# DeepMETv2/DeepMETv2

Measured on AMD Instinct MI355X. Metric: events/sec (4.5k PF cands, k=16), higher is better.
Workload: dtype f32

## Files before the change

deepmetv2_amd/build.py:

```python
from __future__ import annotations

import concurrent.futures as cf
import os
import shutil
import subprocess
import sys

PKG_DIR = os.path.dirname(os.path.abspath(__file__))
CSRC = os.path.join(PKG_DIR, "csrc")
OBJ_DIR = os.path.join(CSRC, "_obj")
LIB_PATH = os.path.join(PKG_DIR, "libdmet_hip.so")
SOURCES = ["knn.hip", "radius.hip", "edgeconv.hip", "edgemlp.hip", "misc.hip", "dense.hip", "encoder.hip", "norm.hip", "edgeconv_bwd.hip",
           "head.hip", "finalize.hip", "pool.hip",
           "edgemlp_f32.hip", "edgemlp_bf16.hip", "edgeconv_sum.hip", "gravnet.hip", "attention.hip", "fps.hip", "interpolate.hip",
           "pointnet.hip", "gat.hip", "segment.hip", "multi_aggr.hip", "weighted_sum.hip", "event_norm.hip", "select.hip",
           "voxel.hip", "edge_match.hip", "components.hip", "condense.hip"]
HEADERS = [os.path.join(CSRC, h) for h in ("common.h", "bn_affine.h", "knn_common.h", "knn_filter.h", "knn_key64.h", "knn_tile_schedule.h",
                                           "nls_body.h",
                                           "edgemlp_fused.h", "row_softmax.h", "score_key.h")] + \
          [os.path.join(PKG_DIR, "..", "include", "dmet.h")]
ARCH = "gfx950"
CXXFLAGS = ["-O3", "-std=c++17", "-fPIC", f"--offload-arch={ARCH}", "-ffp-contract=off", "-Wall",
            "-Wno-unused-function", "-DNDEBUG"]


def _hipcc() -> str:
    exe = shutil.which("hipcc") or "/opt/rocm/bin/hipcc"
    if not os.path.exists(exe):
        raise RuntimeError("hipcc not found: cannot build libdmet_hip.so")
    return exe


def _stale(target: str, deps) -> bool:
    if not os.path.exists(target):
        return True
    t = os.path.getmtime(target)
    return any(os.path.getmtime(d) > t for d in deps if os.path.exists(d))


def _compile(src: str, force: bool) -> str:
    obj = os.path.join(OBJ_DIR, os.path.splitext(src)[0] + ".o")
    path = os.path.join(CSRC, src)
    if force or _stale(obj, [path] + HEADERS):
        cmd = [_hipcc()] + CXXFLAGS + ["-c", path, "-o", obj]
        subprocess.check_call(cmd)
    return obj


def build_hip(force: bool = False, verbose: bool = False) -> str:
    os.makedirs(OBJ_DIR, exist_ok=True)
    with cf.ThreadPoolExecutor(max_workers=min(4, len(SOURCES))) as ex:
        objs = list(ex.map(lambda s: _compile(s, force), SOURCES))
    if force or _stale(LIB_PATH, objs):
        cmd = [_hipcc(), "-shared", "-fPIC", f"--offload-arch={ARCH}", "-o", LIB_PATH] + objs
        if verbose:
            print(" ".join(cmd))
        subprocess.check_call(cmd)
    return LIB_PATH


if __name__ == "__main__":
    print(build_hip(force="--force" in sys.argv, verbose=True))
```

deepmetv2_amd/csrc/encoder.hip:

```cpp
#include <stdlib.h>

#include "bn_affine.h"
#include "common.h"

namespace dmet {
namespace {

typedef float f32x16 __attribute__((ext_vector_type(16)));

#define ENC_PARAMS                                                                                                  \
    const float *__restrict__ Wc, const float *__restrict__ bc, const float *__restrict__ Wk,                      \
        const float *__restrict__ bk, const float *__restrict__ Wa, const float *__restrict__ ba,                  \
        const float *__restrict__ Echg, const float *__restrict__ Epdg, const float *__restrict__ Epv
#define ENC_ARGS Wc, bc, Wk, bk, Wa, ba, Echg, Epdg, Epv

__device__ __forceinline__ float elu(float z) { return z > 0.0f ? z : (__expf(z) - 1.0f); }

__device__ __forceinline__ void cat_indices(const int64_t *__restrict__ xcat, const float *__restrict__ row, int64_t i,
                                            int &ichg, int &ipdg, int &ipv)
{
    long long c = xcat ? xcat[i * 3 + 0] : (long long)row[8];
    const long long chg = xcat ? xcat[i * 3 + 1] : (long long)row[9];
    const long long pv = xcat ? xcat[i * 3 + 2] : (long long)row[10];
    c = c < 0 ? -c : c;
    const long long table[7] = {1, 2, 11, 13, 22, 130, 211};
#pragma unroll
    for (int t = 0; t < 7; ++t) c = (c == table[t]) ? (long long)t : c;
    ipdg = (int)min(max(c, 0ll), 6ll);
    ichg = (int)min(max(chg + 1, 0ll), 2ll);
    ipv = (int)min(max(pv, 0ll), 7ll);
}

__device__ __forceinline__ void encode_node(ENC_PARAMS, const float (&xc)[8], int ichg, int ipdg, int ipv,
                                            float (&cat24)[24], float (&z1)[16], float (&z2)[16], float (&joint)[32],
                                            float (&z3)[32])
{
#pragma unroll
    for (int e = 0; e < 8; ++e) {
        cat24[e] = Echg[ichg * 8 + e];
        cat24[8 + e] = Epdg[ipdg * 8 + e];
        cat24[16 + e] = Epv[ipv * 8 + e];
    }
#pragma unroll
    for (int o = 0; o < 16; ++o) {
        float a = bc[o];
#pragma unroll
        for (int f = 0; f < 8; ++f) a = __builtin_fmaf(Wc[o * 8 + f], xc[f], a);
        z1[o] = a;
        float b = bk[o];
#pragma unroll
        for (int f = 0; f < 24; ++f) b = __builtin_fmaf(Wk[o * 24 + f], cat24[f], b);
        z2[o] = b;
    }
#pragma unroll
    for (int o = 0; o < 16; ++o) { joint[o] = elu(z2[o]); joint[16 + o] = elu(z1[o]); }
#pragma unroll
    for (int o = 0; o < 32; ++o) {
        float a = ba[o];
#pragma unroll
        for (int f = 0; f < 32; ++f) a = __builtin_fmaf(Wa[o * 32 + f], joint[f], a);
        z3[o] = a;
    }
}

__global__ __launch_bounds__(256, 2) void encode_fwd_kernel(const float *__restrict__ x, int64_t x_stride,
                                                          const int64_t *__restrict__ xcat, int64_t N,
                                                          ENC_PARAMS, float *__restrict__ h)
{
    const int64_t i = (int64_t)blockIdx.x * blockDim.x + threadIdx.x;
    if (i >= N) return;
    const float *row = x + i * x_stride;
    float xc[8];
#pragma unroll
    for (int f = 0; f < 8; ++f) xc[f] = row[f];
    int ichg, ipdg, ipv;
    cat_indices(xcat, row, i, ichg, ipdg, ipv);
    float cat24[24], z1[16], z2[16], joint[32], z3[32];
    encode_node(ENC_ARGS, xc, ichg, ipdg, ipv, cat24, z1, z2, joint, z3);
    float4 *o = reinterpret_cast<float4 *>(h + i * 32);
#pragma unroll
    for (int c = 0; c < 8; ++c)
        o[c] = make_float4(elu(z3[4 * c]), elu(z3[4 * c + 1]), elu(z3[4 * c + 2]), elu(z3[4 * c + 3]));
}

__global__ __launch_bounds__(256) void encode_fwd_mfma_kernel(const float *__restrict__ x, int64_t x_stride,
                                                               const int64_t *__restrict__ xcat, int64_t N, ENC_PARAMS,
                                                               float *__restrict__ h)
{
    const int lane = threadIdx.x & 63, r = lane & 31, hh = lane >> 5;
    const int64_t wave = (int64_t)blockIdx.x * (blockDim.x >> 6) + __builtin_amdgcn_readfirstlane((int)(threadIdx.x >> 6));
    const int64_t nwaves = (int64_t)gridDim.x * (blockDim.x >> 6);
    const int64_t ntiles = (N + 31) / 32;
    float w12[16], w3[16], b12[16], b3[16];
#pragma unroll
    for (int s = 0; s < 16; ++s) {
        const int f = (s & 3) + 8 * (s >> 2) + 4 * hh;
        const float *src = r < 16 ? Wk + r * 24 + min(f, 23) : Wc + (r - 16) * 8 + max(f - 24, 0);
        const bool keep = r < 16 ? f < 24 : f >= 24;
        const float a = *src;
        w12[s] = keep ? a : 0.0f;
        w3[s] = Wa[r * 32 + f];
        const float *bsrc = f < 16 ? bk + f : bc + (f - 16);
        b12[s] = *bsrc;
        b3[s] = ba[f];
    }
    struct Raw { float c[4]; long long k0, k1, k2; };
    auto load_raw = [&](const int64_t tile, Raw &q) __attribute__((always_inline)) {
        const int64_t node = tile * 32 + r;
        const int64_t i = node < N ? node : N - 1;
        const float *row = x + i * x_stride;
#pragma unroll
        for (int u = 0; u < 4; ++u) q.c[u] = row[4 * hh + u];
        if (xcat) { q.k0 = xcat[i * 3 + 0]; q.k1 = xcat[i * 3 + 1]; q.k2 = xcat[i * 3 + 2]; }
        else { q.k0 = (long long)row[8]; q.k1 = (long long)row[9]; q.k2 = (long long)row[10]; }
    };
    auto load_tables = [&](const Raw &q, float (&in)[16]) __attribute__((always_inline)) {
        long long c = q.k0 < 0 ? -q.k0 : q.k0;
        const long long table[7] = {1, 2, 11, 13, 22, 130, 211};
#pragma unroll
        for (int t = 0; t < 7; ++t) c = (c == table[t]) ? (long long)t : c;
        const int ipdg = (int)min(max(c, 0ll), 6ll), ichg = (int)min(max(q.k1 + 1, 0ll), 2ll), ipv = (int)min(max(q.k2, 0ll), 7ll);
        const float4 e0 = *reinterpret_cast<const float4 *>(Echg + ichg * 8 + 4 * hh);
        const float4 e1 = *reinterpret_cast<const float4 *>(Epdg + ipdg * 8 + 4 * hh);
        const float4 e2 = *reinterpret_cast<const float4 *>(Epv + ipv * 8 + 4 * hh);
        in[0] = e0.x; in[1] = e0.y; in[2] = e0.z; in[3] = e0.w; in[4] = e1.x; in[5] = e1.y; in[6] = e1.z; in[7] = e1.w;
        in[8] = e2.x; in[9] = e2.y; in[10] = e2.z; in[11] = e2.w;
#pragma unroll
        for (int u = 0; u < 4; ++u) in[12 + u] = q.c[u];
    };
    Raw raw;
    float in[16], nxt[16];
    if (wave < ntiles) { load_raw(wave, raw); load_tables(raw, in); }
    if (wave + nwaves < ntiles) load_raw(wave + nwaves, raw);
    for (int64_t tile = wave; tile < ntiles; tile += nwaves) {
        const int64_t node = tile * 32 + r;
        if (tile + nwaves < ntiles) load_tables(raw, nxt);
        if (tile + 2 * nwaves < ntiles) load_raw(tile + 2 * nwaves, raw);
        f32x16 acc;
#pragma unroll
        for (int e = 0; e < 16; ++e) acc[e] = b12[e];
#pragma unroll
        for (int s = 0; s < 16; ++s) acc = __builtin_amdgcn_mfma_f32_32x32x2f32(w12[s], in[s], acc, 0, 0, 0);
        float joint[16];
#pragma unroll
        for (int e = 0; e < 16; ++e) joint[e] = elu(acc[e]);
#pragma unroll
        for (int e = 0; e < 16; ++e) acc[e] = b3[e];
#pragma unroll
        for (int s = 0; s < 16; ++s) acc = __builtin_amdgcn_mfma_f32_32x32x2f32(w3[s], joint[s], acc, 0, 0, 0);
        if (node < N) {
            float4 *o = reinterpret_cast<float4 *>(h + node * 32 + 4 * hh);
#pragma unroll
            for (int g = 0; g < 4; ++g)
                o[2 * g] = make_float4(elu(acc[4 * g]), elu(acc[4 * g + 1]), elu(acc[4 * g + 2]), elu(acc[4 * g + 3]));
        }
#pragma unroll
        for (int u = 0; u < 16; ++u) in[u] = nxt[u];
    }
}

constexpr int kEncTiles = 3;
constexpr int kEncBwdWaves = 4;
constexpr int kEncPartial = kEncTiles * 1024 + 64;

__device__ __forceinline__ void enc_wave_sync()
{
    __builtin_amdgcn_fence(__ATOMIC_RELEASE, "wavefront");
    __builtin_amdgcn_wave_barrier();
    __builtin_amdgcn_fence(__ATOMIC_ACQUIRE, "wavefront");
}

__device__ __forceinline__ void tile_mma(f32x16 &acc, const float *__restrict__ A, const float *__restrict__ Bm, int lane)
{
    const int c = lane & 31, hh = lane >> 5;
#pragma unroll 8
    for (int s = 0; s < 32; ++s) {
        const int node = 2 * s + hh;
        acc = __builtin_amdgcn_mfma_f32_32x32x2f32(A[node * 33 + c], Bm[node * 33 + c], acc, 0, 0, 0);
    }
}

__device__ __forceinline__ void tile_mma_onehot(f32x16 &acc, const int *__restrict__ packed, const float *__restrict__ Bm,
                                                int lane)
{
    const int c = lane & 31, hh = lane >> 5;
    int sh, mask, tgt;
    if (c < 3) { sh = 0; mask = 3; tgt = c; }
    else if (c < 10) { sh = 2; mask = 7; tgt = c - 3; }
    else if (c < 18) { sh = 5; mask = 7; tgt = c - 10; }
    else { sh = 0; mask = 0; tgt = 1; }
#pragma unroll 8
    for (int s = 0; s < 32; ++s) {
        const int node = 2 * s + hh;
        const float a = (((packed[node] >> sh) & mask) == tgt) ? 1.0f : 0.0f;
        acc = __builtin_amdgcn_mfma_f32_32x32x2f32(a, Bm[node * 33 + c], acc, 0, 0, 0);
    }
}

__device__ __forceinline__ float column_half_sum(const float *__restrict__ A, int lane)
{
    const int c = lane & 31, hh = lane >> 5;
    float s = 0.0f;
#pragma unroll 8
    for (int n = 0; n < 32; ++n) s += A[(hh * 32 + n) * 33 + c];
    return s;
}

__global__ __launch_bounds__(64 * kEncBwdWaves, 2) void encode_bwd_kernel(const float *__restrict__ x, int64_t x_stride,
                                                                          const int64_t *__restrict__ xcat, int64_t N,
                                                                          ENC_PARAMS, const float *__restrict__ gh,
                                                                          const float *__restrict__ hout,
                                                                          int64_t nodes_per_wave,
                                                                          float *__restrict__ partial)
{
    __shared__ float bufA[kEncBwdWaves][64 * 33];
    __shared__ float bufB[kEncBwdWaves][64 * 33];
    __shared__ int bufI[kEncBwdWaves][64];
    const int lane = threadIdx.x & 63, wv = __builtin_amdgcn_readfirstlane(threadIdx.x >> 6);
    float *A = bufA[wv], *Bm = bufB[wv];
    int *packed = bufI[wv];
    const int64_t wave = (int64_t)blockIdx.x * kEncBwdWaves + wv;
    const int64_t lo = wave * nodes_per_wave, hi = min(N, lo + nodes_per_wave);
    f32x16 acc[kEncTiles];
#pragma unroll
    for (int t = 0; t < kEncTiles; ++t)
#pragma unroll
        for (int e = 0; e < 16; ++e) acc[t][e] = 0.0f;
    float bias3 = 0.0f, bias21 = 0.0f;

    for (int64_t base = lo; base < hi; base += 64) {
        int zero = 0;
        asm volatile("" : "+s"(zero));
        const float *__restrict__ wc = Wc + zero, *__restrict__ wk = Wk + zero, *__restrict__ wa = Wa + zero,
                                  *__restrict__ pbc = bc + zero, *__restrict__ pbk = bk + zero;
        const int64_t i = base + lane;
        const bool live = i < hi;
        const int64_t ii = live ? i : (hi - 1);
        const float *row = x + ii * x_stride;
        float xc[8];
#pragma unroll
        for (int f = 0; f < 8; ++f) xc[f] = row[f];
        int ichg, ipdg, ipv;
        cat_indices(xcat, row, ii, ichg, ipdg, ipv);
// ... 128 lines not shown
{
    const int c = lane & 31, hh = lane >> 5;
    float s = 0.0f;
#pragma unroll 8
    for (int n = 0; n < 16; ++n) s += A[(hh * 16 + n) * 33 + c];
    return s;
}

struct EncBnBwd {
    const float *gamma, *mean, *invstd, *mean_g, *mean_gx;
};

template <bool BNB = false>
__global__ __launch_bounds__(64 * kEncBwdWaves, 2) void encode_bwd_mfma_kernel(const float *__restrict__ x, int64_t x_stride,
                                                                               const int64_t *__restrict__ xcat, int64_t N,
                                                                               ENC_PARAMS, const float *__restrict__ gh,
                                                                               const float *__restrict__ hout,
                                                                               int64_t ,
                                                                               float *__restrict__ partial,
                                                                               EncBnBwd bnb = EncBnBwd{})
{
    __shared__ float bufA[kEncBwdWaves][64 * 33];
    __shared__ float bufB[kEncBwdWaves][64 * 33];
    __shared__ int bufI[kEncBwdWaves][64];
    const int lane = threadIdx.x & 63, wv = __builtin_amdgcn_readfirstlane(threadIdx.x >> 6);
    const int r = lane & 31, hh = lane >> 5;
    float *A = bufA[wv], *Bm = bufB[wv];
    int *packed = bufI[wv];
    const int64_t wave = (int64_t)blockIdx.x * kEncBwdWaves + wv, nwaves = (int64_t)gridDim.x * kEncBwdWaves;
    const int64_t ntiles = (N + 31) / 32, hi = N;
    float w12[16], w3t[16], w12t[16], b12[16];
#pragma unroll
    for (int s = 0; s < 16; ++s) {
        const int f = (s & 3) + 8 * (s >> 2) + 4 * hh;
        {
            const float *src = r < 16 ? Wk + r * 24 + min(f, 23) : Wc + (r - 16) * 8 + max(f - 24, 0);
            const bool keep = r < 16 ? f < 24 : f >= 24;
            const float a = *src;
            w12[s] = keep ? a : 0.0f;
        }
        w3t[s] = Wa[f * 32 + r];
        {
            const float *src = f < 16 ? Wk + f * 24 + min(r, 23) : Wc + (f - 16) * 8 + max(r - 24, 0);
            const bool keep = f < 16 ? r < 24 : r >= 24;
            const float a = *src;
            w12t[s] = keep ? a : 0.0f;
        }
        const float *bsrc = f < 16 ? bk + f : bc + (f - 16);
        b12[s] = *bsrc;
    }
    f32x16 acc[kEncTiles];
#pragma unroll
    for (int t = 0; t < kEncTiles; ++t)
#pragma unroll
        for (int e = 0; e < 16; ++e) acc[t][e] = 0.0f;
    float bias3 = 0.0f, bias21 = 0.0f;

    struct Raw { float c[4]; long long k0, k1, k2; };
    auto load_raw = [&](const int64_t tile, Raw &q) __attribute__((always_inline)) {
        const int64_t nd = tile * 32 + r;
        const int64_t i = nd < N ? nd : N - 1;
        const float *row = x + i * x_stride;
#pragma unroll
        for (int u = 0; u < 4; ++u) q.c[u] = row[4 * hh + u];
        if (xcat) { q.k0 = xcat[i * 3 + 0]; q.k1 = xcat[i * 3 + 1]; q.k2 = xcat[i * 3 + 2]; }
        else { q.k0 = (long long)row[8]; q.k1 = (long long)row[9]; q.k2 = (long long)row[10]; }
    };
    auto load_tables = [&](const Raw &q, float (&in)[16], int &pk) __attribute__((always_inline)) {
        long long c = q.k0 < 0 ? -q.k0 : q.k0;
        const long long table[7] = {1, 2, 11, 13, 22, 130, 211};
#pragma unroll
        for (int t = 0; t < 7; ++t) c = (c == table[t]) ? (long long)t : c;
        const int ipdg = (int)min(max(c, 0ll), 6ll), ichg = (int)min(max(q.k1 + 1, 0ll), 2ll), ipv = (int)min(max(q.k2, 0ll), 7ll);
        pk = ichg | (ipdg << 2) | (ipv << 5);
        const float4 e0 = *reinterpret_cast<const float4 *>(Echg + ichg * 8 + 4 * hh);
        const float4 e1 = *reinterpret_cast<const float4 *>(Epdg + ipdg * 8 + 4 * hh);
        const float4 e2 = *reinterpret_cast<const float4 *>(Epv + ipv * 8 + 4 * hh);
        in[0] = e0.x; in[1] = e0.y; in[2] = e0.z; in[3] = e0.w; in[4] = e1.x; in[5] = e1.y; in[6] = e1.z; in[7] = e1.w;
        in[8] = e2.x; in[9] = e2.y; in[10] = e2.z; in[11] = e2.w;
#pragma unroll
        for (int u = 0; u < 4; ++u) in[12 + u] = q.c[u];
    };
    Raw raw;
    float in[16], nxt[16];
    int pk = 0, pk_nxt = 0;
    if (wave < ntiles) { load_raw(wave, raw); load_tables(raw, in, pk); }
    if (wave + nwaves < ntiles) load_raw(wave + nwaves, raw);
    for (int64_t tile = wave; tile < ntiles; tile += nwaves) {
        const int64_t node = tile * 32 + r;
        const bool live = node < hi;
        const int64_t ii = live ? node : (hi - 1);
        if (tile + nwaves < ntiles) load_tables(raw, nxt, pk_nxt);
        if (tile + 2 * nwaves < ntiles) load_raw(tile + 2 * nwaves, raw);
        if (hh == 0) packed[r] = pk;
        float gz[16];
        {
            const float4 *gp = reinterpret_cast<const float4 *>(gh + ii * 32 + 4 * hh);
            const float4 *hp = reinterpret_cast<const float4 *>(hout + ii * 32 + 4 * hh);
#pragma unroll
            for (int g = 0; g < 4; ++g) {
                float4 gv = gp[2 * g];
                const float4 hv = hp[2 * g];
                if constexpr (BNB) {
                    const int c0 = 8 * g + 4 * hh;
                    const float4 ga = *reinterpret_cast<const float4 *>(bnb.gamma + c0), mu = *reinterpret_cast<const float4 *>(bnb.mean + c0);
                    const float4 is = *reinterpret_cast<const float4 *>(bnb.invstd + c0), mg = *reinterpret_cast<const float4 *>(bnb.mean_g + c0);
                    const float4 mx = *reinterpret_cast<const float4 *>(bnb.mean_gx + c0);
                    gv = bn_bwd4(gv, hv, ga, mu, is, mg, mx);
                }
                const float gg[4] = {gv.x, gv.y, gv.z, gv.w}, hh4[4] = {hv.x, hv.y, hv.z, hv.w};
#pragma unroll
                for (int u = 0; u < 4; ++u) {
                    const float d = hh4[u] > 0.0f ? 1.0f : (hh4[u] + 1.0f);
                    gz[4 * g + u] = live ? gg[u] * d : 0.0f;
                }
            }
        }
        f32x16 c1;
#pragma unroll
        for (int e = 0; e < 16; ++e) c1[e] = b12[e];
#pragma unroll
        for (int s = 0; s < 16; ++s) c1 = __builtin_amdgcn_mfma_f32_32x32x2f32(w12[s], in[s], c1, 0, 0, 0);
        float joint[16];
#pragma unroll
        for (int e = 0; e < 16; ++e) joint[e] = elu(c1[e]);
#pragma unroll
        for (int e = 0; e < 16; ++e) {
            const int ch = (e & 3) + 8 * (e >> 2) + 4 * hh;
            A[r * 33 + ch] = gz[e];
            Bm[r * 33 + ch] = joint[e];
        }
        enc_lds_sync();
        tile_mma32(acc[0], A, Bm, lane);
        bias3 += column_half_sum32(A, lane);
        f32x16 c2;
#pragma unroll
        for (int e = 0; e < 16; ++e) c2[e] = 0.0f;
#pragma unroll
        for (int s = 0; s < 16; ++s) c2 = __builtin_amdgcn_mfma_f32_32x32x2f32(w3t[s], gz[s], c2, 0, 0, 0);
        float gj[16];
#pragma unroll
        for (int e = 0; e < 16; ++e) gj[e] = c2[e] * (joint[e] > 0.0f ? 1.0f : (joint[e] + 1.0f));
        enc_lds_sync();
#pragma unroll
        for (int e = 0; e < 16; ++e) {
            const int ch = (e & 3) + 8 * (e >> 2) + 4 * hh;
            A[r * 33 + ch] = gj[e];
            Bm[r * 33 + ch] = in[e];
        }
        enc_lds_sync();
        tile_mma32(acc[1], A, Bm, lane);
        bias21 += column_half_sum32(A, lane);
        f32x16 c3;
#pragma unroll
        for (int e = 0; e < 16; ++e) c3[e] = 0.0f;
#pragma unroll
        for (int s = 0; s < 16; ++s) c3 = __builtin_amdgcn_mfma_f32_32x32x2f32(w12t[s], gj[s], c3, 0, 0, 0);
        enc_lds_sync();
#pragma unroll
        for (int e = 0; e < 16; ++e) {
            const int ch = (e & 3) + 8 * (e >> 2) + 4 * hh;
            Bm[r * 33 + ch] = ch < 24 ? c3[e] : 0.0f;
        }
        enc_lds_sync();
        tile_mma_onehot32(acc[2], packed, Bm, lane);
        enc_lds_sync();
#pragma unroll
        for (int u = 0; u < 16; ++u) in[u] = nxt[u];
        pk = pk_nxt;
    }
    const int c = lane & 31;
    __syncthreads();
#pragma unroll
    for (int e = 0; e < 16; ++e) {
        const int rr = (e & 3) + 8 * (e >> 2) + 4 * hh;
        A[rr * 32 + c] = acc[0][e];
        A[1024 + rr * 32 + c] = acc[2][e];
        Bm[rr * 32 + c] = acc[1][e];
    }
    const float b3 = bias3 + __shfl_xor(bias3, 32), b21 = bias21 + __shfl_xor(bias21, 32);
    if (hh == 0) { Bm[1024 + c] = b3; Bm[1024 + 32 + c] = b21; }
    __syncthreads();
    float *out = partial + (int64_t)blockIdx.x * kEncPartial;
    for (int i = threadIdx.x; i < kEncPartial; i += 64 * kEncBwdWaves) {
        const float *src = i < 1024 ? &bufA[0][i] : i < 2048 ? &bufB[0][i - 1024] : i < 3072 ? &bufA[0][i - 1024]
                                                                                              : &bufB[0][i - 2048];
        float t = src[0];
#pragma unroll
        for (int w = 1; w < kEncBwdWaves; ++w) t += src[w * 64 * 33];
        out[i] = t;
    }
}

struct EncGrads {
    float *Wc, *bc, *Wk, *bk, *Wa, *ba, *Echg, *Epdg, *Epv;
};

__global__ __launch_bounds__(1024) void encode_bwd_finalize_kernel(const float *__restrict__ partial, int64_t nwaves,
                                                                    EncGrads g)
{
    __shared__ float red[32][33];
    const int e = threadIdx.x & 31, grp = threadIdx.x >> 5;
    const int idx = blockIdx.x * 32 + e;
    float s = 0.0f;
#pragma unroll 8
    for (int64_t w = grp; w < nwaves; w += 32) s += partial[w * kEncPartial + idx];
    red[grp][e] = s;
    __syncthreads();
    if (grp != 0) return;
    s = 0.0f;
#pragma unroll
    for (int q = 0; q < 32; ++q) s += red[q][e];
    const int t = idx / 1024, r = (idx % 1024) / 32, c = idx % 32;
    if (t == 0) g.Wa[r * 32 + c] = s;
    else if (t == 1) {
        if (r < 16 && c < 24) g.Wk[r * 24 + c] = s;
        else if (r >= 16 && c >= 24) g.Wc[(r - 16) * 8 + (c - 24)] = s;
    } else if (t == 2) {
        if (r < 3 && c < 8) g.Echg[r * 8 + c] = s;
        else if (r >= 3 && r < 10 && c >= 8 && c < 16) g.Epdg[(r - 3) * 8 + (c - 8)] = s;
        else if (r >= 10 && r < 18 && c >= 16 && c < 24) g.Epv[(r - 10) * 8 + (c - 16)] = s;
    } else if (r == 0) g.ba[c] = s;
    else if (c < 16) g.bk[c] = s;
    else g.bc[c - 16] = s;
}

inline int64_t enc_nodes_per_wave(int64_t N, int64_t *nwaves)
{
    const int64_t target_waves = 2048;
    int64_t npw = (N + target_waves - 1) / target_waves;
#ifdef DMET_ENC_NPW_UP
    npw = (npw + 63) / 64 * 64;
#else
    npw = npw / 64 * 64;
#endif
    if (npw < 64) npw = 64;
    int64_t nw = (N + npw - 1) / npw;
    nw = (nw + kEncBwdWaves - 1) / kEncBwdWaves * kEncBwdWaves;
    *nwaves = nw;
    return npw;
}

thread_local EncBnBwd g_enc_bnb{nullptr, nullptr, nullptr, nullptr, nullptr};
thread_local bool g_enc_bnb_done = false;

}
}

using namespace dmet;

extern "C" int dmet_encode_fwd_f32(const float *x, int64_t x_stride, const int64_t *xcat, int64_t N, const float *Wc, const float *bc,
                                   const float *Wk, const float *bk, const float *Wa, const float *ba,
                                   const float *Echg, const float *Epdg, const float *Epv, float *h,
                                   dmet_stream_t stream)
{
    DMET_REQUIRE(N >= 0 && x_stride >= 8, "dmet_encode_fwd_f32: bad sizes");
    if (N == 0) return 0;
    DMET_REQUIRE(x && Wc && bc && Wk && bk && Wa && ba && Echg && Epdg && Epv && h, "dmet_encode_fwd_f32: null pointer");
    DMET_REQUIRE(xcat || x_stride >= 11, "dmet_encode_fwd_f32: x_cat == NULL needs rows of at least 11 columns (x_stride=%lld)", (long long)x_stride);
    DMET_REQUIRE(aligned16(h), "dmet_encode_fwd_f32: h must be 16-B aligned");
    const int64_t blocks = (N + 255) / 256;
    DMET_REQUIRE(blocks < (1ll << 31), "dmet_encode_fwd_f32: too many nodes");
    const int form = env_is("DMET_ENCODER_FWD", "valu") ? 0 : 1;
    if (form == 1 && aligned16(Echg) && aligned16(Epdg) && aligned16(Epv)) {
        const int64_t tiles = (N + 31) / 32;
        int64_t grid = (tiles + 3) / 4;
        int gmax = 512;
        if (const char *e = getenv("DMET_ENC_GRID")) { gmax = atoi(e); if (gmax < 1) gmax = 512; }
        if (grid > gmax) grid = gmax;
        hipLaunchKernelGGL(encode_fwd_mfma_kernel, dim3((unsigned)grid), dim3(256), 0, as_stream(stream), x, x_stride, xcat, N,
                           ENC_ARGS, h);
        DMET_LAUNCH_CHECK("encode_fwd_mfma_kernel");
        return 0;
    }
    hipLaunchKernelGGL(encode_fwd_kernel, dim3((unsigned)blocks), dim3(256), 0, as_stream(stream), x, x_stride, xcat, N, ENC_ARGS, h);
    DMET_LAUNCH_CHECK("encode_fwd_kernel");
    return 0;
}

extern "C" size_t dmet_encode_bwd_workspace_bytes(int64_t N)
{
    if (N <= 0) return 0;
    int64_t nw;
    (void)enc_nodes_per_wave(N, &nw);
    return sizeof(float) * (size_t)nw * kEncPartial + 512;
}

extern "C" int dmet_encode_bwd_f32(const float *x, int64_t x_stride, const int64_t *xcat, int64_t N, const float *Wc, const float *bc,
                                   const float *Wk, const float *bk, const float *Wa, const float *ba,
                                   const float *Echg, const float *Epdg, const float *Epv, const float *h,
                                   const float *g_h, float *gWc, float *gbc, float *gWk, float *gbk, float *gWa,
                                   float *gba, float *gEchg, float *gEpdg, float *gEpv, void *ws, size_t ws_bytes,
                                   dmet_stream_t stream)
{
    DMET_REQUIRE(N > 0 && x_stride >= 8, "dmet_encode_bwd_f32: bad sizes");
    DMET_REQUIRE((xcat || x_stride >= 11) && x && Wc && bc && Wk && bk && Wa && ba && Echg && Epdg && Epv && h && g_h && gWc && gbc && gWk && gbk &&
                     gWa && gba && gEchg && gEpdg && gEpv && ws,
                 "dmet_encode_bwd_f32: null pointer");
    DMET_REQUIRE(ws_bytes >= dmet_encode_bwd_workspace_bytes(N), "dmet_encode_bwd_f32: workspace too small");
    DMET_REQUIRE(aligned16(h) && aligned16(g_h), "dmet_encode_bwd_f32: h / g_h must be 16-B aligned");
    int64_t nw;
    const int64_t npw = enc_nodes_per_wave(N, &nw);
    float *partial = reinterpret_cast<float *>((reinterpret_cast<uintptr_t>(ws) + 255u) & ~(uintptr_t)255u);
    hipStream_t st = as_stream(stream);
    const int form = env_is("DMET_ENCODER_BWD", "valu") ? 0 : 1;
    int64_t nparts = nw / kEncBwdWaves;
    if (form == 1 && aligned16(Echg) && aligned16(Epdg) && aligned16(Epv) && aligned16(g_h) && aligned16(h)) {
        const int64_t tiles = (N + 31) / 32;
        int64_t grid = (tiles + kEncBwdWaves - 1) / kEncBwdWaves;
        if (grid > 512) grid = 512;
        if (grid > nparts) grid = nparts;
        nparts = grid;
        if (g_enc_bnb.gamma)
            hipLaunchKernelGGL(encode_bwd_mfma_kernel<true>, dim3((unsigned)grid), dim3(64 * kEncBwdWaves), 0, st, x, x_stride, xcat,
                               N, ENC_ARGS, g_h, h, npw, partial, g_enc_bnb);
        else
            hipLaunchKernelGGL(encode_bwd_mfma_kernel<false>, dim3((unsigned)grid), dim3(64 * kEncBwdWaves), 0, st, x, x_stride,
                               xcat, N, ENC_ARGS, g_h, h, npw, partial, EncBnBwd{});
        g_enc_bnb_done = g_enc_bnb.gamma != nullptr;
    } else {
        hipLaunchKernelGGL(encode_bwd_kernel, dim3((unsigned)(nw / kEncBwdWaves)), dim3(64 * kEncBwdWaves), 0, st, x, x_stride,
                           xcat, N, ENC_ARGS, g_h, h, npw, partial);
    }
    DMET_LAUNCH_CHECK("encode_bwd_kernel");
    EncGrads gr{gWc, gbc, gWk, gbk, gWa, gba, gEchg, gEpdg, gEpv};
    static_assert(kEncPartial % 32 == 0, "finalize blocks own 32 elements");
    static_assert(kEncPartial == kEncPartialFloats, "csrc/finalize.hip sums the same partial layout");
    if (defer_push(DeferDesc{kDeferEncoder, partial, nparts, {gWc, gbc, gWk, gbk, gWa, gba, gEchg, gEpdg, gEpv}})) return 0;
    hipLaunchKernelGGL(encode_bwd_finalize_kernel, dim3(kEncPartial / 32), dim3(1024), 0, st, partial, nparts, gr);
    DMET_LAUNCH_CHECK("encode_bwd_finalize_kernel");
    return 0;
}

extern "C" int dmet_encode_bn_bwd_f32(const float *x, int64_t x_stride, const int64_t *xcat, int64_t N, const float *Wc,
                                      const float *bc, const float *Wk, const float *bk, const float *Wa, const float *ba,
                                      const float *Echg, const float *Epdg, const float *Epv, const float *h,
                                      const float *g_y, const float *bn_gamma, const float *bn_mean, const float *bn_invstd,
                                      const float *bn_mean_g, const float *bn_mean_gx, float *gWc, float *gbc, float *gWk,
                                      float *gbk, float *gWa, float *gba, float *gEchg, float *gEpdg, float *gEpv,
                                      int *fused, void *ws, size_t ws_bytes, dmet_stream_t stream)
{
    DMET_REQUIRE(fused, "dmet_encode_bn_bwd_f32: fused is null");
    *fused = 0;
    DMET_REQUIRE(bn_gamma && bn_mean && bn_invstd && bn_mean_g && bn_mean_gx, "dmet_encode_bn_bwd_f32: null pointer");
    const bool ok = !env_is("DMET_ENCODER_BWD", "valu") && N > 0 && aligned16(Echg) && aligned16(Epdg) && aligned16(Epv) && aligned16(g_y) &&
                    aligned16(h) && aligned16(bn_gamma) && aligned16(bn_mean) && aligned16(bn_invstd) && aligned16(bn_mean_g) &&
                    aligned16(bn_mean_gx);
    if (!ok) return 0;
    g_enc_bnb = EncBnBwd{bn_gamma, bn_mean, bn_invstd, bn_mean_g, bn_mean_gx};
    g_enc_bnb_done = false;
    const int rc = dmet_encode_bwd_f32(x, x_stride, xcat, N, Wc, bc, Wk, bk, Wa, ba, Echg, Epdg, Epv, h, g_y, gWc, gbc, gWk, gbk, gWa,
                                       gba, gEchg, gEpdg, gEpv, ws, ws_bytes, stream);
    const bool done = g_enc_bnb_done;
    g_enc_bnb = EncBnBwd{nullptr, nullptr, nullptr, nullptr, nullptr};
    g_enc_bnb_done = false;
    if (rc == 0 && !done) {
        set_error("dmet_encode_bn_bwd_f32: the matrix-core backward it was checked for did not run");
        return -22;
    }
    *fused = rc == 0 ? 1 : 0;
    return rc;
}
```

Measured before the change: 53370.

## Add two-stream interleaved MFMA encoder kernels and move bwd prefetch later

Adds forward and backward encoder kernels in which each wavefront processes two node tiles at once, interleaving their MFMA chains with the ELU/VALU work of the other stream to hide dependency latency. A shared node-tile schedule header is introduced. The new kernels are opt-in via DMET_NODE_STREAMS=2. The existing backward kernel is also changed to prefetch the next tile's tables after the LDS stage instead of holding a separate nxt buffer, which saves registers but makes the loads later in the loop.

```diff
diff --git a/deepmetv2_amd/build.py b/deepmetv2_amd/build.py
--- a/deepmetv2_amd/build.py
+++ b/deepmetv2_amd/build.py
@@ -16,7 +16,7 @@
            "pointnet.hip", "gat.hip", "segment.hip", "multi_aggr.hip", "weighted_sum.hip", "event_norm.hip", "select.hip",
            "voxel.hip", "edge_match.hip", "components.hip", "condense.hip"]
 HEADERS = [os.path.join(CSRC, h) for h in ("common.h", "bn_affine.h", "knn_common.h", "knn_filter.h", "knn_key64.h", "knn_tile_schedule.h",
-                                           "nls_body.h",
+                                           "nls_body.h", "node_tile_schedule.h",
                                            "edgemlp_fused.h", "row_softmax.h", "score_key.h")] + \
           [os.path.join(PKG_DIR, "..", "include", "dmet.h")]
 ARCH = "gfx950"
diff --git a/deepmetv2_amd/csrc/encoder.hip b/deepmetv2_amd/csrc/encoder.hip
--- a/deepmetv2_amd/csrc/encoder.hip
+++ b/deepmetv2_amd/csrc/encoder.hip
@@ -2,6 +2,7 @@
 
 #include "bn_affine.h"
 #include "common.h"
+#include "node_tile_schedule.h"
 
 namespace dmet {
 namespace {
@@ -159,6 +160,151 @@
     }
 }
 
+struct EncRaw { float c[4]; long long k0, k1, k2; };
+
+__device__ __forceinline__ void enc_load_raw(const float *__restrict__ x, int64_t x_stride, const int64_t *__restrict__ xcat,
+                                             int64_t N, int64_t tile, int r, int hh, EncRaw &q)
+{
+    const int64_t i = node_row(tile, r, N);
+    const float *row = x + i * x_stride;
+#pragma unroll
+    for (int u = 0; u < 4; ++u) q.c[u] = row[4 * hh + u];
+    if (xcat) { q.k0 = xcat[i * 3 + 0]; q.k1 = xcat[i * 3 + 1]; q.k2 = xcat[i * 3 + 2]; }
+    else { q.k0 = (long long)row[8]; q.k1 = (long long)row[9]; q.k2 = (long long)row[10]; }
+}
+
+__device__ __forceinline__ void enc_load_tables(const float *__restrict__ Echg, const float *__restrict__ Epdg,
+                                                const float *__restrict__ Epv, int hh, const EncRaw &q, float (&in)[16], int &pk)
+{
+    long long c = q.k0 < 0 ? -q.k0 : q.k0;
+    const long long table[7] = {1, 2, 11, 13, 22, 130, 211};
+#pragma unroll
+    for (int t = 0; t < 7; ++t) c = (c == table[t]) ? (long long)t : c;
+    const int ipdg = (int)min(max(c, 0ll), 6ll), ichg = (int)min(max(q.k1 + 1, 0ll), 2ll), ipv = (int)min(max(q.k2, 0ll), 7ll);
+    pk = ichg | (ipdg << 2) | (ipv << 5);
+    const float4 e0 = *reinterpret_cast<const float4 *>(Echg + ichg * 8 + 4 * hh);
+    const float4 e1 = *reinterpret_cast<const float4 *>(Epdg + ipdg * 8 + 4 * hh);
+    const float4 e2 = *reinterpret_cast<const float4 *>(Epv + ipv * 8 + 4 * hh);
+    in[0] = e0.x; in[1] = e0.y; in[2] = e0.z; in[3] = e0.w; in[4] = e1.x; in[5] = e1.y; in[6] = e1.z; in[7] = e1.w;
+    in[8] = e2.x; in[9] = e2.y; in[10] = e2.z; in[11] = e2.w;
+#pragma unroll
+    for (int u = 0; u < 4; ++u) in[12 + u] = q.c[u];
+}
+
+__device__ __forceinline__ void enc_pin(float &v)
+{
+    asm volatile("" : "+v"(v));
+    __builtin_amdgcn_sched_barrier(0);
+}
+
+__device__ __forceinline__ float enc_elu_here(float z)
+{
+    asm volatile("" : "+v"(z));
+    float a = elu(z);
+    enc_pin(a);
+    return a;
+}
+
+__device__ __forceinline__ void enc_pin_acc(f32x16 &c)
+{
+    asm volatile("" : "+a"(c));
+}
+
+__device__ __forceinline__ f32x16 enc_splat(const float (&b)[16])
+{
+    f32x16 a;
+#pragma unroll
+    for (int e = 0; e < 16; ++e) a[e] = b[e];
+    return a;
+}
+
+__global__ __launch_bounds__(256) void encode_fwd_mfma2_kernel(const float *__restrict__ x, int64_t x_stride,
+                                                                const int64_t *__restrict__ xcat, int64_t N, ENC_PARAMS,
+                                                                float *__restrict__ h)
+{
+    constexpr int S = kNodeStreams;
+    static_assert(S == 2, "the stages below are written out for two streams");
+    const int lane = threadIdx.x & 63, r = lane & 31, hh = lane >> 5;
+    const int64_t wavefront = (int64_t)blockIdx.x * (blockDim.x >> 6) + __builtin_amdgcn_readfirstlane((int)(threadIdx.x >> 6));
+    const int64_t nw = (int64_t)gridDim.x * (blockDim.x >> 6) * S;
+    const int64_t ntiles = node_tile_count(N);
+    float w12[16], w3[16], b12[16], b3[16];
+#pragma unroll
+    for (int s = 0; s < 16; ++s) {
+        const int f = (s & 3) + 8 * (s >> 2) + 4 * hh;
+        const float *src = r < 16 ? Wk + r * 24 + min(f, 23) : Wc + (r - 16) * 8 + max(f - 24, 0);
+        const bool keep = r < 16 ? f < 24 : f >= 24;
+        const float a = *src;
+        w12[s] = keep ? a : 0.0f;
+        w3[s] = Wa[r * 32 + f];
+        const float *bsrc = f < 16 ? bk + f : bc + (f - 16);
+        b12[s] = *bsrc;
+        b3[s] = ba[f];
+    }
+    int64_t w[S];
+    EncRaw raw[S];
+    float in[S][16], nxt[S][16];
+    int pk_unused;
+#pragma unroll
+    for (int q = 0; q < S; ++q) {
+        w[q] = node_stream_wave(wavefront, q, S);
+#pragma unroll
+        for (int u = 0; u < 16; ++u) { in[q][u] = 0.0f; nxt[q][u] = 0.0f; }
+        if (node_stream_has(w[q], 0, nw, ntiles)) enc_load_raw(x, x_stride, xcat, N, node_stream_tile(w[q], 0, nw), r, hh, raw[q]);
+    }
+#pragma unroll
+    for (int q = 0; q < S; ++q) {
+        if (node_stream_has(w[q], 0, nw, ntiles)) enc_load_tables(Echg, Epdg, Epv, hh, raw[q], in[q], pk_unused);
+        if (node_stream_has(w[q], 1, nw, ntiles)) enc_load_raw(x, x_stride, xcat, N, node_stream_tile(w[q], 1, nw), r, hh, raw[q]);
+    }
+    const int64_t rounds = node_rounds(w[0], nw, ntiles);
+    for (int64_t j = 0; j < rounds; ++j) {
+#pragma unroll
+        for (int q = 0; q < S; ++q) {
+            if (node_stream_has(w[q], j + 1, nw, ntiles)) enc_load_tables(Echg, Epdg, Epv, hh, raw[q], nxt[q], pk_unused);
+            if (node_stream_has(w[q], j + kNodePrefetch, nw, ntiles))
+                enc_load_raw(x, x_stride, xcat, N, node_stream_tile(w[q], j + kNodePrefetch, nw), r, hh, raw[q]);
+        }
+        f32x16 c1[S], c2[S];
+        float joint[S][16];
+        c1[0] = enc_splat(b12);
+#pragma unroll
+        for (int s = 0; s < 16; ++s) c1[0] = __builtin_amdgcn_mfma_f32_32x32x2f32(w12[s], in[0][s], c1[0], 0, 0, 0);
+        c1[1] = enc_splat(b12);
+#pragma unroll
+        for (int s = 0; s < 16; ++s) {
+            c1[1] = __builtin_amdgcn_mfma_f32_32x32x2f32(w12[s], in[1][s], c1[1], 0, 0, 0);
+            joint[0][s] = elu(c1[0][s]);
+        }
+        c2[0] = enc_splat(b3);
+#pragma unroll
+        for (int s = 0; s < 16; ++s) {
+            c2[0] = __builtin_amdgcn_mfma_f32_32x32x2f32(w3[s], joint[0][s], c2[0], 0, 0, 0);
+            joint[1][s] = elu(c1[1][s]);
+        }
+        c2[1] = enc_splat(b3);
+        float out0[16];
+#pragma unroll
+        for (int s = 0; s < 16; ++s) {
+            c2[1] = __builtin_amdgcn_mfma_f32_32x32x2f32(w3[s], joint[1][s], c2[1], 0, 0, 0);
+            out0[s] = elu(c2[0][s]);
+        }
+#pragma unroll
+        for (int q = 0; q < S; ++q) {
+            const int64_t tile = node_stream_tile(w[q], j, nw);
+            if (node_row_live(tile, r, N)) {
+                float4 *o = reinterpret_cast<float4 *>(h + (tile * kNodeTileRows + r) * 32 + 4 * hh);
+#pragma unroll
+                for (int g = 0; g < 4; ++g)
+                    o[2 * g] = q == 0 ? make_float4(out0[4 * g], out0[4 * g + 1], out0[4 * g + 2], out0[4 * g + 3])
+                                      : make_float4(elu(c2[1][4 * g]), elu(c2[1][4 * g + 1]), elu(c2[1][4 * g + 2]), elu(c2[1][4 * g + 3]));
+            }
+#pragma unroll
+            for (int u = 0; u < 16; ++u) in[q][u] = nxt[q][u];
+        }
+    }
+}
+
 constexpr int kEncTiles = 3;
 constexpr int kEncBwdWaves = 4;
 constexpr int kEncPartial = kEncTiles * 1024 + 64;
@@ -453,16 +599,14 @@
         for (int u = 0; u < 4; ++u) in[12 + u] = q.c[u];
     };
     Raw raw;
-    float in[16], nxt[16];
-    int pk = 0, pk_nxt = 0;
+    float in[16];
+    int pk = 0;
     if (wave < ntiles) { load_raw(wave, raw); load_tables(raw, in, pk); }
     if (wave + nwaves < ntiles) load_raw(wave + nwaves, raw);
     for (int64_t tile = wave; tile < ntiles; tile += nwaves) {
         const int64_t node = tile * 32 + r;
         const bool live = node < hi;
         const int64_t ii = live ? node : (hi - 1);
-        if (tile + nwaves < ntiles) load_tables(raw, nxt, pk_nxt);
-        if (tile + 2 * nwaves < ntiles) load_raw(tile + 2 * nwaves, raw);
         if (hh == 0) packed[r] = pk;
         float gz[16];
         {
@@ -520,6 +664,8 @@
             Bm[r * 33 + ch] = in[e];
         }
         enc_lds_sync();
+        if (tile + nwaves < ntiles) load_tables(raw, in, pk);
+        if (tile + 2 * nwaves < ntiles) load_raw(tile + 2 * nwaves, raw);
         tile_mma32(acc[1], A, Bm, lane);
         bias21 += column_half_sum32(A, lane);
         f32x16 c3;
@@ -536,9 +682,6 @@
         enc_lds_sync();
         tile_mma_onehot32(acc[2], packed, Bm, lane);
         enc_lds_sync();
-#pragma unroll
-        for (int u = 0; u < 16; ++u) in[u] = nxt[u];
-        pk = pk_nxt;
     }
     const int c = lane & 31;
     __syncthreads();
@@ -559,6 +702,252 @@
         float t = src[0];
 #pragma unroll
         for (int w = 1; w < kEncBwdWaves; ++w) t += src[w * 64 * 33];
+        out[i] = t;
+    }
+}
+
+template <int T>
+__device__ __forceinline__ void tile_mma32_streams(f32x16 (&acc)[kNodeStreams][kEncTiles], float (&bias)[kNodeStreams],
+                                                   float *const (&A)[kNodeStreams], float *const (&Bm)[kNodeStreams], int lane)
+{
+    const int c = lane & 31, hh = lane >> 5;
+    float cs[kNodeStreams];
+#pragma unroll
+    for (int q = 0; q < kNodeStreams; ++q) cs[q] = 0.0f;
+#pragma unroll
+    for (int s = 0; s < 16; ++s)
+#pragma unroll
+        for (int q = 0; q < kNodeStreams; ++q) {
+            const int node = 2 * s + hh;
+            acc[q][T] = __builtin_amdgcn_mfma_f32_32x32x2f32(A[q][node * 33 + c], Bm[q][node * 33 + c], acc[q][T], 0, 0, 0);
+            cs[q] += A[q][(hh * 16 + s) * 33 + c];
+        }
+#pragma unroll
+    for (int q = 0; q < kNodeStreams; ++q) bias[q] += cs[q];
+}
+
+__device__ __forceinline__ void tile_mma_onehot32_streams(f32x16 (&acc)[kNodeStreams][kEncTiles], int *const (&packed)[kNodeStreams],
+                                                          float *const (&Bm)[kNodeStreams], int lane)
+{
+    const int c = lane & 31, hh = lane >> 5;
+    int sh, mask, tgt;
+    if (c < 3) { sh = 0; mask = 3; tgt = c; }
+    else if (c < 10) { sh = 2; mask = 7; tgt = c - 3; }
+    else if (c < 18) { sh = 5; mask = 7; tgt = c - 10; }
+    else { sh = 0; mask = 0; tgt = 1; }
+#pragma unroll
+    for (int s = 0; s < 16; ++s)
+#pragma unroll
+        for (int q = 0; q < kNodeStreams; ++q) {
+            const int node = 2 * s + hh;
+            const float a = (((packed[q][node] >> sh) & mask) == tgt) ? 1.0f : 0.0f;
+            acc[q][2] = __builtin_amdgcn_mfma_f32_32x32x2f32(a, Bm[q][node * 33 + c], acc[q][2], 0, 0, 0);
+        }
+}
+
+template <bool BNB = false>
+__global__ __launch_bounds__(64 * kEncBwdWaves / kNodeStreams, 1) void encode_bwd_mfma2_kernel(
+    const float *__restrict__ x, int64_t x_stride, const int64_t *__restrict__ xcat, int64_t N, ENC_PARAMS,
+    const float *__restrict__ gh, const float *__restrict__ hout, float *__restrict__ partial, EncBnBwd bnb = EncBnBwd{})
+{
+    constexpr int S = kNodeStreams;
+    static_assert(S == 2 && kEncBwdWaves == kNodeBwdGroupStreams, "two wavefronts of two streams stand for the four of a partial");
+    __shared__ float bufA[kEncBwdWaves][64 * 33];
+    __shared__ float bufB[kEncBwdWaves][64 * 33];
+    __shared__ int bufI[kEncBwdWaves][64];
+    const int lane = threadIdx.x & 63, wv = __builtin_amdgcn_readfirstlane(threadIdx.x >> 6);
+    const int r = lane & 31, hh = lane >> 5;
+    const int64_t wavefront = (int64_t)blockIdx.x * (kEncBwdWaves / S) + wv;
+    const int64_t nw = (int64_t)gridDim.x * kEncBwdWaves;
+    const int64_t ntiles = node_tile_count(N);
+    float *A[S], *Bm[S];
+    int *packed[S];
+    int64_t w[S];
+#pragma unroll
+    for (int q = 0; q < S; ++q) {
+        A[q] = bufA[S * wv + q]; Bm[q] = bufB[S * wv + q]; packed[q] = bufI[S * wv + q];
+        w[q] = node_stream_wave(wavefront, q, S);
+    }
+    float w12[16], w3t[16], w12t[16], b12[16];
+#pragma unroll
+    for (int s = 0; s < 16; ++s) {
+        const int f = (s & 3) + 8 * (s >> 2) + 4 * hh;
+        {
+            const float *src = r < 16 ? Wk + r * 24 + min(f, 23) : Wc + (r - 16) * 8 + max(f - 24, 0);
+            const bool keep = r < 16 ? f < 24 : f >= 24;
+            const float a = *src;
+            w12[s] = keep ? a : 0.0f;
+        }
+        w3t[s] = Wa[f * 32 + r];
+        {
+            const float *src = f < 16 ? Wk + f * 24 + min(r, 23) : Wc + (f - 16) * 8 + max(r - 24, 0);
+            const bool keep = f < 16 ? r < 24 : r >= 24;
+            const float a = *src;
+            w12t[s] = keep ? a : 0.0f;
+        }
+        const float *bsrc = f < 16 ? bk + f : bc + (f - 16);
+        b12[s] = *bsrc;
+    }
+    f32x16 acc[S][kEncTiles];
+    float bias3[S], bias21[S];
+    EncRaw raw[S];
+    float in[S][16];
+    int pk[S];
+#pragma unroll
+    for (int q = 0; q < S; ++q) {
+#pragma unroll
+        for (int t = 0; t < kEncTiles; ++t)
+#pragma unroll
+            for (int e = 0; e < 16; ++e) acc[q][t][e] = 0.0f;
+        bias3[q] = 0.0f; bias21[q] = 0.0f; pk[q] = 0;
+#pragma unroll
+        for (int u = 0; u < 16; ++u) in[q][u] = 0.0f;
+        if (node_stream_has(w[q], 0, nw, ntiles)) enc_load_raw(x, x_stride, xcat, N, node_stream_tile(w[q], 0, nw), r, hh, raw[q]);
+    }
+#pragma unroll
+    for (int q = 0; q < S; ++q) {
+        if (node_stream_has(w[q], 0, nw, ntiles)) enc_load_tables(Echg, Epdg, Epv, hh, raw[q], in[q], pk[q]);
+        if (node_stream_has(w[q], 1, nw, ntiles)) enc_load_raw(x, x_stride, xcat, N, node_stream_tile(w[q], 1, nw), r, hh, raw[q]);
+    }
+    const int64_t rounds = node_rounds(w[0], nw, ntiles);
+    for (int64_t j = 0; j < rounds; ++j) {
+        float gz[S][16];
+        int zero = 0;
+        asm volatile("" : "+s"(zero));
+        const EncBnBwd bn{bnb.gamma + zero, bnb.mean + zero, bnb.invstd + zero, bnb.mean_g + zero, bnb.mean_gx + zero};
+#pragma unroll
+        for (int q = 0; q < S; ++q) {
+            if (hh == 0) packed[q][r] = pk[q];
+        }
+        bool live[S];
+        const float4 *gp[S], *hp[S];
+#pragma unroll
+        for (int q = 0; q < S; ++q) {
+            const int64_t tile = node_stream_tile(w[q], j, nw);
+            live[q] = node_row_live(tile, r, N);
+            const int64_t ii = node_row(tile, r, N);
+            gp[q] = reinterpret_cast<const float4 *>(gh + ii * 32 + 4 * hh);
+            hp[q] = reinterpret_cast<const float4 *>(hout + ii * 32 + 4 * hh);
+        }
+#pragma unroll
+        for (int g = 0; g < 4; ++g) {
+            float4 ga, mu, is, mg, mx;
+            if constexpr (BNB) {
+                const int c0 = 8 * g + 4 * hh;
+                ga = *reinterpret_cast<const float4 *>(bn.gamma + c0); mu = *reinterpret_cast<const float4 *>(bn.mean + c0);
+                is = *reinterpret_cast<const float4 *>(bn.invstd + c0); mg = *reinterpret_cast<const float4 *>(bn.mean_g + c0);
+                mx = *reinterpret_cast<const float4 *>(bn.mean_gx + c0);
+            }
+#pragma unroll
+            for (int q = 0; q < S; ++q) {
+                float4 gv = gp[q][2 * g];
+                const float4 hv = hp[q][2 * g];
+                if constexpr (BNB) gv = bn_bwd4(gv, hv, ga, mu, is, mg, mx);
+                const float gg[4] = {gv.x, gv.y, gv.z, gv.w}, hh4[4] = {hv.x, hv.y, hv.z, hv.w};
+#pragma unroll
+                for (int u = 0; u < 4; ++u) {
+                    const float d = hh4[u] > 0.0f ? 1.0f : (hh4[u] + 1.0f);
+                    gz[q][4 * g + u] = live[q] ? gg[u] * d : 0.0f;
+                }
+            }
+        }
+        f32x16 c1[S], c2[S], c3[S];
+        float joint[S][16], gj[S][16];
+        c1[0] = enc_splat(b12);
+#pragma unroll
+        for (int s = 0; s < 16; ++s) c1[0] = __builtin_amdgcn_mfma_f32_32x32x2f32(w12[s], in[0][s], c1[0], 0, 0, 0);
+        c1[1] = enc_splat(b12);
+#pragma unroll
+        for (int s = 0; s < 16; ++s) {
+            c1[1] = __builtin_amdgcn_mfma_f32_32x32x2f32(w12[s], in[1][s], c1[1], 0, 0, 0);
+            enc_pin_acc(c1[1]);
+            joint[0][s] = enc_elu_here(c1[0][s]);
+        }
+#pragma unroll
+        for (int e = 0; e < 16; ++e) c2[0][e] = 0.0f;
+#pragma unroll
+        for (int s = 0; s < 16; ++s) {
+            c2[0] = __builtin_amdgcn_mfma_f32_32x32x2f32(w3t[s], gz[0][s], c2[0], 0, 0, 0);
+            enc_pin_acc(c2[0]);
+            joint[1][s] = enc_elu_here(c1[1][s]);
+        }
+#pragma unroll
+        for (int e = 0; e < 16; ++e) c2[1][e] = 0.0f;
+#pragma unroll
+        for (int s = 0; s < 16; ++s) {
+            c2[1] = __builtin_amdgcn_mfma_f32_32x32x2f32(w3t[s], gz[1][s], c2[1], 0, 0, 0);
+            const int ch = (s & 3) + 8 * (s >> 2) + 4 * hh;
+            A[0][r * 33 + ch] = gz[0][s];
+            Bm[0][r * 33 + ch] = joint[0][s];
+            __builtin_amdgcn_sched_barrier(0);
+        }
+#pragma unroll
+        for (int e = 0; e < 16; ++e) {
+            const int ch = (e & 3) + 8 * (e >> 2) + 4 * hh;
+            A[1][r * 33 + ch] = gz[1][e];
+            Bm[1][r * 33 + ch] = joint[1][e];
+        }
+        enc_lds_sync();
+        tile_mma32_streams<0>(acc, bias3, A, Bm, lane);
+#pragma unroll
+        for (int q = 0; q < S; ++q)
+#pragma unroll
+            for (int e = 0; e < 16; ++e) gj[q][e] = c2[q][e] * (joint[q][e] > 0.0f ? 1.0f : (joint[q][e] + 1.0f));
+        enc_lds_sync();
+#pragma unroll
+        for (int q = 0; q < S; ++q) {
+#pragma unroll
+            for (int e = 0; e < 16; ++e) c3[q][e] = 0.0f;
+#pragma unroll
+            for (int s = 0; s < 16; ++s) {
+                c3[q] = __builtin_amdgcn_mfma_f32_32x32x2f32(w12t[s], gj[q][s], c3[q], 0, 0, 0);
+                const int ch = (s & 3) + 8 * (s >> 2) + 4 * hh;
+                A[q][r * 33 + ch] = gj[q][s];
+                Bm[q][r * 33 + ch] = in[q][s];
+            }
+        }
+        enc_lds_sync();
+#pragma unroll
+        for (int q = 0; q < S; ++q) {
+            if (node_stream_has(w[q], j + 1, nw, ntiles)) enc_load_tables(Echg, Epdg, Epv, hh, raw[q], in[q], pk[q]);
+            if (node_stream_has(w[q], j + kNodePrefetch, nw, ntiles))
+                enc_load_raw(x, x_stride, xcat, N, node_stream_tile(w[q], j + kNodePrefetch, nw), r, hh, raw[q]);
+        }
+        tile_mma32_streams<1>(acc, bias21, A, Bm, lane);
+        enc_lds_sync();
+#pragma unroll
+        for (int q = 0; q < S; ++q)
+#pragma unroll
+            for (int e = 0; e < 16; ++e) {
+                const int ch = (e & 3) + 8 * (e >> 2) + 4 * hh;
+                Bm[q][r * 33 + ch] = ch < 24 ? c3[q][e] : 0.0f;
+            }
+        enc_lds_sync();
+        tile_mma_onehot32_streams(acc, packed, Bm, lane);
+        enc_lds_sync();
+    }
+    const int c = lane & 31;
+    __syncthreads();
+#pragma unroll
+    for (int q = 0; q < S; ++q) {
+#pragma unroll
+        for (int e = 0; e < 16; ++e) {
+            const int rr = (e & 3) + 8 * (e >> 2) + 4 * hh;
+            A[q][rr * 32 + c] = acc[q][0][e];
+            A[q][1024 + rr * 32 + c] = acc[q][2][e];
+            Bm[q][rr * 32 + c] = acc[q][1][e];
+        }
+        const float b3 = bias3[q] + __shfl_xor(bias3[q], 32), b21 = bias21[q] + __shfl_xor(bias21[q], 32);
+        if (hh == 0) { Bm[q][1024 + c] = b3; Bm[q][1024 + 32 + c] = b21; }
+    }
+    __syncthreads();
+    float *out = partial + (int64_t)blockIdx.x * kEncPartial;
+    for (int i = threadIdx.x; i < kEncPartial; i += 64 * kEncBwdWaves / S) {
+        const float *src = i < 1024 ? &bufA[0][i] : i < 2048 ? &bufB[0][i - 1024] : i < 3072 ? &bufA[0][i - 1024]
+                                                                                              : &bufB[0][i - 2048];
+        float t = src[0];
+#pragma unroll
+        for (int wq = 1; wq < kEncBwdWaves; ++wq) t += src[wq * 64 * 33];
         out[i] = t;
     }
 }
@@ -612,6 +1001,15 @@
     return npw;
 }
 
+inline bool node_two_streams() { return env_is("DMET_NODE_STREAMS", "2"); }
+
+inline int64_t node_grid_cap(const char *name, int64_t dflt)
+{
+    const char *e = getenv(name);
+    const int64_t v = e ? atoll(e) : 0;
+    return v >= 1 && v < dflt ? v : dflt;
+}
+
 thread_local EncBnBwd g_enc_bnb{nullptr, nullptr, nullptr, nullptr, nullptr};
 thread_local bool g_enc_bnb_done = false;
 
@@ -634,13 +1032,18 @@
     DMET_REQUIRE(blocks < (1ll << 31), "dmet_encode_fwd_f32: too many nodes");
     const int form = env_is("DMET_ENCODER_FWD", "valu") ? 0 : 1;
     if (form == 1 && aligned16(Echg) && aligned16(Epdg) && aligned16(Epv)) {
-        const int64_t tiles = (N + 31) / 32;
-        int64_t grid = (tiles + 3) / 4;
-        int gmax = 512;
-        if (const char *e = getenv("DMET_ENC_GRID")) { gmax = atoi(e); if (gmax < 1) gmax = 512; }
-        if (grid > gmax) grid = gmax;
-        hipLaunchKernelGGL(encode_fwd_mfma_kernel, dim3((unsigned)grid), dim3(256), 0, as_stream(stream), x, x_stride, xcat, N,
-                           ENC_ARGS, h);
+        const int64_t tiles = node_tile_count(N);
+        const bool two = node_two_streams();
+        const int gdef = two ? 256 : 512;
+        int gmax = gdef;
+        if (const char *e = getenv("DMET_ENC_GRID")) { gmax = atoi(e); if (gmax < 1) gmax = gdef; }
+        const int64_t grid = node_grid(tiles, two ? kNodeFwdGroupStreams : 4, gmax);
+        if (two)
+            hipLaunchKernelGGL(encode_fwd_mfma2_kernel, dim3((unsigned)grid), dim3(256), 0, as_stream(stream), x, x_stride, xcat, N,
+                               ENC_ARGS, h);
+        else
+            hipLaunchKernelGGL(encode_fwd_mfma_kernel, dim3((unsigned)grid), dim3(256), 0, as_stream(stream), x, x_stride, xcat, N,
+                               ENC_ARGS, h);
         DMET_LAUNCH_CHECK("encode_fwd_mfma_kernel");
         return 0;
     }
@@ -677,16 +1080,22 @@
     const int form = env_is("DMET_ENCODER_BWD", "valu") ? 0 : 1;
     int64_t nparts = nw / kEncBwdWaves;
     if (form == 1 && aligned16(Echg) && aligned16(Epdg) && aligned16(Epv) && aligned16(g_h) && aligned16(h)) {
-        const int64_t tiles = (N + 31) / 32;
-        int64_t grid = (tiles + kEncBwdWaves - 1) / kEncBwdWaves;
-        if (grid > 512) grid = 512;
-        if (grid > nparts) grid = nparts;
+        const int64_t cap = node_grid_cap("DMET_ENC_BWD_GRID", 512);
+        const int64_t grid = node_grid(node_tile_count(N), kNodeBwdGroupStreams, cap < nparts ? cap : nparts);
         nparts = grid;
-        if (g_enc_bnb.gamma)
-            hipLaunchKernelGGL(encode_bwd_mfma_kernel<true>, dim3((unsigned)grid), dim3(64 * kEncBwdWaves), 0, st, x, x_stride, xcat,
+        const bool two = node_two_streams();
+        const dim3 block(two ? 64 * kEncBwdWaves / kNodeStreams : 64 * kEncBwdWaves);
+        if (g_enc_bnb.gamma && two)
+            hipLaunchKernelGGL(encode_bwd_mfma2_kernel<true>, dim3((unsigned)grid), block, 0, st, x, x_stride, xcat, N, ENC_ARGS,
+                               g_h, h, partial, g_enc_bnb);
+        else if (two)
+            hipLaunchKernelGGL(encode_bwd_mfma2_kernel<false>, dim3((unsigned)grid), block, 0, st, x, x_stride, xcat, N, ENC_ARGS,
+                               g_h, h, partial, EncBnBwd{});
+        else if (g_enc_bnb.gamma)
+            hipLaunchKernelGGL(encode_bwd_mfma_kernel<true>, dim3((unsigned)grid), block, 0, st, x, x_stride, xcat,
                                N, ENC_ARGS, g_h, h, npw, partial, g_enc_bnb);
         else
-            hipLaunchKernelGGL(encode_bwd_mfma_kernel<false>, dim3((unsigned)grid), dim3(64 * kEncBwdWaves), 0, st, x, x_stride,
+            hipLaunchKernelGGL(encode_bwd_mfma_kernel<false>, dim3((unsigned)grid), block, 0, st, x, x_stride,
                                xcat, N, ENC_ARGS, g_h, h, npw, partial, EncBnBwd{});
         g_enc_bnb_done = g_enc_bnb.gamma != nullptr;
     } else {
diff --git a/deepmetv2_amd/csrc/node_tile_schedule.h b/deepmetv2_amd/csrc/node_tile_schedule.h
--- /dev/null
+++ b/deepmetv2_amd/csrc/node_tile_schedule.h
@@ -0,0 +1,43 @@
+#pragma once
+
+#include <stdint.h>
+
+#if defined(__HIPCC__) || defined(__CUDACC__)
+#define DMET_NODE_SCHED_FN __host__ __device__ inline
+#else
+#define DMET_NODE_SCHED_FN inline
+#endif
+
+constexpr int kNodeTileRows = 32;
+constexpr int kNodeStreams = 2;
+constexpr int kNodePrefetch = 2;
+constexpr int kNodeBwdGroupStreams = 4;
+constexpr int kNodeFwdGroupStreams = 4 * kNodeStreams;
+
+DMET_NODE_SCHED_FN constexpr int64_t node_tile_count(int64_t N) { return (N + kNodeTileRows - 1) / kNodeTileRows; }
+
+DMET_NODE_SCHED_FN constexpr int64_t node_stream_wave(int64_t v, int s, int streams) { return v * streams + s; }
+
+DMET_NODE_SCHED_FN constexpr int64_t node_stream_tile(int64_t w, int64_t j, int64_t nw) { return w + j * nw; }
+DMET_NODE_SCHED_FN constexpr bool node_stream_has(int64_t w, int64_t j, int64_t nw, int64_t ntiles)
+{
+    return node_stream_tile(w, j, nw) < ntiles;
+}
+
+DMET_NODE_SCHED_FN constexpr int64_t node_rounds(int64_t w0, int64_t nw, int64_t ntiles)
+{
+    return ntiles > w0 ? (ntiles - w0 + nw - 1) / nw : 0;
+}
+
+DMET_NODE_SCHED_FN constexpr int64_t node_row(int64_t tile, int r, int64_t N)
+{
+    return tile * kNodeTileRows + r < N ? tile * kNodeTileRows + r : N - 1;
+}
+DMET_NODE_SCHED_FN constexpr bool node_row_live(int64_t tile, int r, int64_t N) { return tile * kNodeTileRows + r < N; }
+
+DMET_NODE_SCHED_FN constexpr int64_t node_grid(int64_t ntiles, int group_streams, int64_t cap)
+{
+    int64_t g = (ntiles + group_streams - 1) / group_streams;
+    if (g > cap) g = cap;
+    return g < 1 ? 1 : g;
+}
```

After: 53350, median of 4. Within noise of the previous version (-0.0%).
